# Elliotshui/ABRSimulator

Measured on AMD Instinct MI355X. Metric: env_steps_per_sec, higher is better.
Workload: dtype f64

## Files before the change

### abrsimulator_amd/csrc/abr_env.hip

```cpp
#include <hip/hip_runtime.h>

#include <climits>
#include <cmath>
#include <cstdarg>
#include <cstdio>
#include <cstdlib>
#include <cstring>
#include <new>
#include <type_traits>
#include <vector>

#include "abr_env.h"

#ifdef ABR_SPLIT_STAMPS
#include "abr_diag_stamps.h"
#else
#define ABR_STAMP(n)
#define ABR_STAMP_INIT()
#define ABR_STAMP_FLUSH()
#define ABR_WG_TIME(slot)
#define ABR_WG_WHERE(role)
#define K3_STAMP_DECL
#define K3_STAMP(n)
#define K3_STAMP_FLUSH()
#endif
#define ABR_RULE_KERNARG_OFFSET 592
#include "abr_lane_jump.h"
#include "abr_tick_tables.h"

static thread_local char g_err[512] = "";

static int fail(int code, const char *fmt, ...) {
    va_list ap;
    va_start(ap, fmt);
    vsnprintf(g_err, sizeof(g_err), fmt, ap);
    va_end(ap);
    return code;
}
#define HIP_TRY(expr)                                                                     \
    do {                                                                                  \
        hipError_t e__ = (expr);                                                          \
        if (e__ != hipSuccess)                                                            \
            return fail(ABR_E_HIP, "%s failed: %s", #expr, hipGetErrorString(e__));       \
    } while (0)

extern "C" int abr_abi_version(void) { return ABR_ABI_VERSION; }
extern "C" const char *abr_last_error(void) { return g_err; }

constexpr double kDt = 0.01;
constexpr int kFlagStartUp = 1, kFlagBufEmpty = 2, kFlagBufFull = 4;
constexpr int kFlagArmed = 8;

struct EnvParams {
    int32_t n_rates, video_length, max_ticks, auto_reset;
    int32_t play_ticks_per_chunk;
    int32_t n_intervals;
    int32_t t_block;
    int32_t n_traces;
    double chunk_length, max_buffer, start_up_length;
    double wr, wv, ws, wl;
    double sd;
    double ladder[ABR_MAX_RATES];
    int64_t n_lanes, lane_id_base;
    const double *G;
    const double *GP;
    const int32_t *interval_tick;
    const int32_t *avail_tick;
    abrx::DrainTab drain;
    const double *traces;
    const int64_t *trace_off;
    const int32_t *trace_len;
    double *buf, *last_bw, *hist_n, *hist_s;
    double *sd_lane, *pt_lane;
    const double *lane_speeds;
    int32_t speed_rows;
    int32_t *pl_left, *play_id;
    double *pt_sum;
    const double *br_table;
    long long *sumk;
    int32_t *k, *chunk_id, *n_su, *n_rb, *n_play, *j, *tpos, *trace_id, *offset0;
    int32_t *last_action, *n_su_obs, *n_rb_obs, *episode_no;
    uint8_t *flags, *done;
    uint8_t *action_hist;
    double *bw_hist;
    double *ep_qoe_terms;
    double *var_run;
    uint32_t *selfcheck_out;
    uint64_t sentinel;
    abrx::SpeedRuleBlock speed_rule;
};
static_assert(offsetof(EnvParams, speed_rule) == ABR_RULE_KERNARG_OFFSET, "abr_lane_jump.h reads the rule at this offset");
static_assert(sizeof(EnvParams) == 880, "the parameter block: 592 bytes + 288 of the speed rule");
static_assert(sizeof(abrx::SpeedRule) == sizeof(abr_speed_rule) &&
              offsetof(abrx::SpeedRule, lat_thr) == offsetof(abr_speed_rule, lat_thr) &&
              offsetof(abrx::SpeedRule, buf_thr) == offsetof(abr_speed_rule, buf_thr) &&
              offsetof(abrx::SpeedRule, speed) == offsetof(abr_speed_rule, speed), "abr_speed_rule: one layout");

constexpr uint32_t kTagMagic = 0x57524241u;
constexpr uint32_t kLayoutRev = 1;
struct WorkspaceTag {
    uint32_t magic, abi_version, layout_rev, n_rates;
    int64_t n_lanes;
    int32_t video_length, max_ticks, n_intervals, reserved_;
    uint64_t total_bytes;
    double chunk_length, interval, speed;
    uint8_t pad_[256 - 72];
};
static_assert(sizeof(WorkspaceTag) == 256, "the tag is one 256-byte block");
static_assert(sizeof(abrx::EpisodeSampler) == sizeof(abr_episode_sampler) &&
              offsetof(abrx::EpisodeSampler, pool) == offsetof(abr_episode_sampler, pool) &&
              offsetof(abrx::EpisodeSampler, n_pool) == offsetof(abr_episode_sampler, n_pool) &&
              offsetof(abrx::EpisodeSampler, offset_span) == offsetof(abr_episode_sampler, offset_span),
              "abr_episode_sampler: one layout");
static_assert(sizeof(abrx::EpisodeLedger) == sizeof(abr_episode_ledger) &&
              offsetof(abrx::EpisodeLedger, base) == offsetof(abr_episode_ledger, base_dev) &&
              offsetof(abrx::EpisodeLedger, rows) == offsetof(abr_episode_ledger, rows),
              "abr_episode_ledger: one layout");

struct abr_env {
    EnvParams p;
    abr_env_config cfg;
    size_t workspace_bytes;
    void *tag_dev;
    WorkspaceTag tag;
    int impl;
    int32_t *mpc_action;
    void *mpc_scratch;
    const double *pending_speeds;
    int32_t pending_speed_rows;
    bool pending_rule_on;
    abrx::SpeedRuleBlock pending_rule;
    bool speeds_dirty;
    const double *pending_br_table;
    bool br_table_dirty;
    bool armed;
    bool sampler_on;
    abrx::EpisodeSampler sampler;
    abrx::EpisodeLedger ledger;
};

static void apply_pending(abr_env *env) {
    if (env->br_table_dirty) { env->p.br_table = env->pending_br_table; env->br_table_dirty = false; }
    if (env->speeds_dirty) {
        env->p.lane_speeds = env->pending_speeds; env->p.speed_rows = env->pending_speed_rows;
        env->p.speed_rule = env->pending_rule;
        if (env->pending_rule_on) { env->p.lane_speeds = env->p.sd_lane; env->p.speed_rows = abrx::kSpeedRowsRule; }
        env->speeds_dirty = false;
    }
}

__device__ inline double chunk_bitrate(const EnvParams &p, int32_t chunk, int32_t rate) {
    return p.br_table ? p.br_table[(int64_t)chunk * p.n_rates + rate] : p.ladder[rate];
// ... 307 lines not shown
            bf = bufB >= max_buffer;
            be = bufB <= 0.0;
            buf = be ? 0.0 : bufB;
            su = su && !(buf >= sul);
            k += running ? 1 : 0;
            const bool next = running && (chunk_id < V) && (k < max_ticks);
            n_su += (next && su) ? 1 : 0;
            n_rb += (next && !su && be) ? 1 : 0;
            const bool call = done_dl && (k >= avail_k) && !bf;
            running = next && !call;
            const bool cross = (k == k_end);
            c = cross ? c_next : c;
            crossed = crossed || cross;
        }
        if (active) {
            s.buf = buf; s.dl = dl; s.c = c; s.k = k; s.chunk_id = chunk_id; s.n_su = n_su;
            s.n_rb = n_rb; s.n_play = n_play; s.n_dl = n_dl; s.avail_k = avail_k;
            s.su = su; s.be = be; s.bf = bf; s.done_dl = done_dl; s.running = running;
            s.sumk += (long long)sk;
            (void)crossed;
        }
    }

    if (touched) {
        lane_store(s, p, i);
        p.n_su_obs[i] = n_su_obs; p.n_rb_obs[i] = n_rb_obs; p.episode_no[i] = episode_no;
        p.last_bw[i] = last_bw; p.hist_n[i] = hist_n; p.hist_s[i] = hist_s; p.var_run[i] = var_run;
        p.done[i] = done;
        if (MODE != 0) {
            for (int32_t t = step_idx; t < n_total; t++) {
                const int64_t o = (int64_t)t * p.n_lanes + i;
                if (reward_out) reward_out[o] = 0.0f;
                if (done_out) done_out[o] = done;
                if ((MODE == 2 || MODE == 4) && actions_out) actions_out[o] = -1;
                if (obs_out)
                    write_obs(s, p, i, obs_out + (int64_t)t * ABR_OBS_DIM * p.n_lanes, last_bw);
            }
        }
    }
}

using abrx::LaneJ;

__device__ inline abrx::Tables make_tables(const EnvParams &p, bool cascade = true) {
    abrx::Tables t;
    t.G = p.G; t.interval_tick = p.interval_tick; t.avail_tick = p.avail_tick;
    t.L = p.chunk_length; t.sd = p.sd; t.max_buffer = p.max_buffer;
    t.start_up_length = p.start_up_length; t.V = p.video_length; t.max_ticks = p.max_ticks;
    t.per_lane_speed = p.lane_speeds != nullptr;
    t.speed_rows = p.lane_speeds ? p.speed_rows : 0;
    t.speed_stride = p.n_lanes; t.speeds = p.lane_speeds;
    t.drain = p.drain;
    if (p.lane_speeds || !cascade) t.drain.n = 0;
#ifdef ABR_NO_DRAIN_CASCADE
    t.drain.n = 0;
#endif
    return t;
}

__device__ inline void lanej_load(LaneJ &s, const EnvParams &p, int64_t i) {
    s.buf = p.buf[i]; s.sumk = p.sumk[i];
    s.k = p.k[i]; s.chunk_id = p.chunk_id[i]; s.n_su = p.n_su[i]; s.n_rb = p.n_rb[i];
    s.n_play = p.n_play[i]; s.cur.j = p.j[i]; s.cur.tpos = p.tpos[i];
    s.last_action = p.last_action[i];
    const uint8_t f = p.flags[i];
    s.su = f & kFlagStartUp; s.be = f & kFlagBufEmpty; s.bf = f & kFlagBufFull;
    const int32_t c = s.chunk_id < p.video_length ? s.chunk_id : p.video_length;
    s.avail_k = p.avail_tick[c];
    if (p.lane_speeds) { s.sd = p.sd_lane[i]; s.pt = p.pt_lane[i]; } else { s.sd = p.sd; s.pt = 0.0; }
    s.lane = i; s.pl_left = 0; s.play_id = 0; s.pt_sum = 0.0;
    if (p.lane_speeds && p.speed_rows >= 2) { s.pl_left = p.pl_left[i]; s.play_id = p.play_id[i]; s.pt_sum = p.pt_sum[i]; }
}

__device__ inline void lanej_store(const LaneJ &s, const EnvParams &p, int64_t i) {
    p.buf[i] = s.buf; p.sumk[i] = s.sumk;
    p.k[i] = s.k; p.chunk_id[i] = s.chunk_id; p.n_su[i] = s.n_su; p.n_rb[i] = s.n_rb;
    p.n_play[i] = s.n_play; p.j[i] = s.cur.j; p.tpos[i] = s.cur.tpos; p.last_action[i] = s.last_action;
    p.flags[i] = (uint8_t)((s.su ? kFlagStartUp : 0) | (s.be ? kFlagBufEmpty : 0) |
                           (s.bf ? kFlagBufFull : 0) | kFlagArmed);
    if (p.lane_speeds) { p.sd_lane[i] = s.sd; p.pt_lane[i] = s.pt; }
    if (p.lane_speeds && p.speed_rows >= 2) { p.pl_left[i] = s.pl_left; p.play_id[i] = s.play_id; p.pt_sum[i] = s.pt_sum; }
}

#ifndef ABR_NO_NT_STORES
#define ABR_OUT(ref, val) __builtin_nontemporal_store((val), &(ref))
#else
#define ABR_OUT(ref, val) ((ref) = (val))
#endif

__device__ inline void write_obs_j(const LaneJ &s, const EnvParams &p, int64_t i, float *obs,
                                   double last_bw) {
    if (!obs) return;
    const int64_t n = p.n_lanes;
    ABR_OUT(obs[ABR_OBS_CHUNK_ID * n + i], (float)s.chunk_id);
    ABR_OUT(obs[ABR_OBS_LAST_BITRATE * n + i], (float)s.last_action);
    ABR_OUT(obs[ABR_OBS_LAST_BANDWIDTH * n + i], (float)last_bw);
    ABR_OUT(obs[ABR_OBS_BUFFER_LEVEL * n + i], (float)s.buf);
    ABR_OUT(obs[ABR_OBS_GLOBAL_TIME * n + i], (float)p.G[s.k]);
    ABR_OUT(obs[ABR_OBS_PLAY_TIME * n + i], (float)(p.lane_speeds ? s.pt : p.GP[s.n_play]));
    ABR_OUT(obs[ABR_OBS_REBUFFER_TIME * n + i], (float)p.G[s.n_rb]);
    ABR_OUT(obs[ABR_OBS_STARTUP_TIME * n + i], (float)p.G[s.n_su]);
}

__device__ inline void write_obs_vals(const LaneJ &s, const EnvParams &p, int64_t i, float *obs, double last_bw,
                                      double g_k, double g_play, double g_rb, double g_su) {
    if (!obs) return;
// ... 187 lines not shown
}

__global__ void observe_f64_kernel(EnvParams p, double *__restrict__ out) {
    const int64_t i = (int64_t)blockIdx.x * blockDim.x + threadIdx.x;
    if (i >= p.n_lanes) return;
    const int64_t n = p.n_lanes;
    out[ABR_F64_GLOBAL_TIME * n + i] = p.G[p.k[i]];
    out[ABR_F64_REBUFFER_TIME * n + i] = p.G[p.n_rb[i]];
    out[ABR_F64_STARTUP_TIME * n + i] = p.G[p.n_su[i]];
    int32_t P = p.play_ticks_per_chunk;
    const bool sched = p.lane_speeds && p.speed_rows >= 2;
    if (p.lane_speeds) {
        double x = 0.0; int32_t a = 0;
        abrx::chain<abrx::STOP_GE>(x, p.sd_lane[i], p.chunk_length, p.max_ticks + 1, a);
        P = a > 0 ? a : 1;
        out[ABR_F64_PLAY_TIME * n + i] = p.pt_lane[i];
        out[ABR_F64_AVERAGE_LATENCY * n + i] =
            sched ? avg_latency_sched(p.pt_lane[i], p.sumk[i], p.pt_sum[i], p.n_play[i])
                  : avg_latency_from(p.sd_lane[i], p.pt_lane[i], p.sumk[i], p.n_play[i]);
    } else {
        out[ABR_F64_PLAY_TIME * n + i] = p.GP[p.n_play[i]];
        out[ABR_F64_AVERAGE_LATENCY * n + i] = lane_avg_latency(p, p.sumk[i], p.n_play[i]);
    }
    out[ABR_F64_BUFFER_LEVEL * n + i] = p.buf[i];
    if (sched) {
        const int32_t pl = p.pl_left[i];
        double x = 0.0; int32_t a = 0;
        abrx::chain<abrx::STOP_GE>(x, p.sd_lane[i], 1.0e300, pl > 0 ? P - pl : 0, a);
        out[ABR_F64_PLAY_LENGTH * n + i] = x;
    } else if (p.lane_speeds) {
        double x = 0.0; int32_t a = 0;
        abrx::chain<abrx::STOP_GE>(x, p.sd_lane[i], 1.0e300, p.n_play[i] % P, a);
        out[ABR_F64_PLAY_LENGTH * n + i] = x;
    } else {
        out[ABR_F64_PLAY_LENGTH * n + i] = p.GP[p.n_play[i] % P];
    }
    out[ABR_F64_LAST_BANDWIDTH * n + i] = p.last_bw[i];
    out[ABR_F64_CHUNK_ID * n + i] = (double)p.chunk_id[i];
    out[ABR_F64_PLAY_ID * n + i] = sched ? (double)p.play_id[i] : (double)(p.n_play[i] / P);
    out[ABR_F64_LAST_BITRATE * n + i] = (double)p.last_action[i];
    out[ABR_F64_FLAGS * n + i] = (double)p.flags[i];
    out[ABR_F64_HIST_N * n + i] = p.hist_n[i];
    out[ABR_F64_HIST_SUM_INV * n + i] = p.hist_s[i];
    out[ABR_F64_TICK * n + i] = (double)p.k[i];
    out[ABR_F64_DOWNLOAD_TIME * n + i] = 0.0;
}

static size_t align_up(size_t x, size_t a) { return (x + a - 1) / a * a; }
static size_t mpc_scratch_bytes_max(size_t n_lanes) {
    return n_lanes * ((size_t)ABR_MAX_HORIZON * sizeof(double) + 2 * sizeof(int32_t));
}

struct Layout {
    size_t G, GP, interval_tick, avail_tick;
    size_t f64_state, i64_state, i32_state, u8_state, action_hist, bw_hist, ep_terms;
    size_t mpc_action, mpc_scratch;
    size_t tag;
    size_t total;
    int32_t max_ticks, n_intervals;
};

static double min_episode_ticks(const abr_env_config *c) {
    return ((double)c->video_length + 1.0) * ceil(c->chunk_length / kDt);
}
static double default_max_ticks(const abr_env_config *c) {
    double per_chunk = ceil(c->chunk_length / kDt);
    double mt = 32.0 * c->video_length * per_chunk;
    if (mt > 16.0e6) mt = 16.0e6;
    if (mt < 2.0 * min_episode_ticks(c)) mt = 2.0 * min_episode_ticks(c);
    if (mt < 1024) mt = 1024;
    return mt;
}

static int validate_cfg(const abr_env_config *c) {
    if (!c) return fail(ABR_E_INVALID, "config is NULL");
    if (c->n_rates < 1 || c->n_rates > ABR_MAX_RATES)
        return fail(ABR_E_INVALID, "n_rates %d outside 1..%d", c->n_rates, ABR_MAX_RATES);
    if (c->video_length < 1 || c->video_length > 65535)
        return fail(ABR_E_INVALID, "video_length %d outside 1..65535", c->video_length);
    if (!(c->chunk_length > 0) || !(c->interval > 0) || !(c->speed > 0))
        return fail(ABR_E_INVALID, "chunk_length, interval and speed must be > 0");
    if (!(c->max_buffer > 0)) return fail(ABR_E_INVALID, "max_buffer must be > 0");
    if (!(c->start_up_length >= 0)) return fail(ABR_E_INVALID, "start_up_length must be >= 0");
    if (c->chunk_length / kDt > 1.0e6)
        return fail(ABR_E_UNSUPPORTED, "chunk_length %g s is more than 1e6 ticks", c->chunk_length);
    for (int r = 0; r < c->n_rates; r++)
        if (!(c->ladder[r] > 0)) return fail(ABR_E_INVALID, "ladder[%d] must be > 0", r);
    return ABR_OK;
}

static int compute_layout(const abr_env_config *c, int64_t n_lanes, Layout *L) {
    int rc = validate_cfg(c);
    if (rc) return rc;
    if (n_lanes < 1) return fail(ABR_E_INVALID, "n_lanes must be >= 1");
    const double mtd = c->max_ticks > 0 ? (double)c->max_ticks : default_max_ticks(c);
    if (mtd > 256.0e6)
        return fail(ABR_E_UNSUPPORTED, "video_length %d x chunk_length %g s needs a %g-entry tick table",
                    c->video_length, c->chunk_length, mtd);
    if (mtd < min_episode_ticks(c))
        return fail(ABR_E_INVALID, "max_ticks %g is below (video_length + 1) * ceil(chunk_length / dt) = %g: "
                    "every lane would end in ABR_DONE_TIMEOUT", mtd, min_episode_ticks(c));
    const int32_t mt = (int32_t)mtd;
    double n_iv = (double)mt * kDt / c->interval + 4.0;
    if (n_iv > 32.0e6)
        return fail(ABR_E_UNSUPPORTED, "interval %g s needs a %g-entry tick table", c->interval, n_iv);
    L->max_ticks = mt;
    L->n_intervals = (int32_t)n_iv;
    size_t o = 0;
    const size_t A = 256;
    size_t N = (size_t)n_lanes, V = (size_t)c->video_length;
    L->G = o; o = align_up(o + sizeof(double) * ((size_t)mt + 2), A);
    L->GP = o; o = align_up(o + sizeof(double) * ((size_t)mt + 2), A);
    L->interval_tick = o; o = align_up(o + sizeof(int32_t) * ((size_t)L->n_intervals + 8), A);
    L->avail_tick = o; o = align_up(o + sizeof(int32_t) * (V + 2), A);
    L->f64_state = o; o = align_up(o + sizeof(double) * 8 * N, A);
    L->i64_state = o; o = align_up(o + sizeof(long long) * 1 * N, A);
    L->i32_state = o; o = align_up(o + sizeof(int32_t) * 15 * N, A);
    L->u8_state = o; o = align_up(o + 2 * N, A);
    L->action_hist = o; o = align_up(o + V * N, A);
    L->bw_hist = o; o = align_up(o + sizeof(double) * V * N, A);
    L->ep_terms = o; o = align_up(o + sizeof(double) * 4 * N, A);
    L->mpc_action = o; o = align_up(o + sizeof(int32_t) * N, A);
    L->mpc_scratch = o; o = align_up(o + mpc_scratch_bytes_max(N), A);
    L->tag = o; o = align_up(o + sizeof(WorkspaceTag), A);
    L->total = o;
    return ABR_OK;
}

extern "C" int abr_env_workspace_bytes(const abr_env_config *cfg, int64_t n_lanes,
                                       size_t *bytes_out) {
    Layout L;
    int rc = compute_layout(cfg, n_lanes, &L);
    if (rc) return rc;
    if (!bytes_out) return fail(ABR_E_INVALID, "bytes_out is NULL");
    *bytes_out = L.total;
    return ABR_OK;
}

extern "C" int abr_env_create(const abr_env_config *cfg, const double *traces_dev,
                              const int64_t *trace_off_dev, const int32_t *trace_len_dev,
                              int32_t n_traces, int64_t n_lanes, void *workspace_dev,
                              size_t workspace_bytes, void *stream, abr_env **env_out) {
    Layout L;
    int rc = compute_layout(cfg, n_lanes, &L);
    if (rc) return rc;
    if (!env_out) return fail(ABR_E_INVALID, "env_out is NULL");
    if (!traces_dev || !trace_off_dev || !trace_len_dev || n_traces < 1)
        return fail(ABR_E_INVALID, "trace arrays missing");
    if (!workspace_dev || ((uintptr_t)workspace_dev & 255))
        return fail(ABR_E_WORKSPACE, "workspace must be non-NULL and 256-B aligned");
    if (workspace_bytes < L.total)
        return fail(ABR_E_WORKSPACE, "workspace has %zu bytes, need %zu", workspace_bytes, L.total);

    const int32_t mt = L.max_ticks;
    abrx::TickTables tt = abrx::build_tick_tables(cfg->interval, cfg->chunk_length, cfg->speed,
                                                  cfg->video_length, mt, L.n_intervals);
    std::vector<double> &G = tt.G, &GP = tt.GP;
    std::vector<int32_t> &itick = tt.interval_tick, &atick = tt.avail_tick;
    const double sd = tt.sd;
    const int32_t P = tt.play_ticks_per_chunk;
    int32_t t_block = tt.min_interval_ticks < 128 ? tt.min_interval_ticks : 128;
    if (t_block < 1) t_block = 1;
    if (P == INT_MAX)
        return fail(ABR_E_UNSUPPORTED, "max_ticks %d too small to play one chunk", mt);

    abr_env *e = new (std::nothrow) abr_env;
    if (!e) return fail(ABR_E_INVALID, "out of host memory");
    memset(e, 0, sizeof(*e));
    e->cfg = *cfg;
    e->impl = 3;
    e->workspace_bytes = L.total;
    EnvParams &p = e->p;
    p.n_rates = cfg->n_rates; p.video_length = cfg->video_length; p.max_ticks = mt;
    p.auto_reset = cfg->auto_reset; p.play_ticks_per_chunk = P; p.n_intervals = L.n_intervals;
    p.t_block = t_block; p.n_traces = n_traces;
    p.chunk_length = cfg->chunk_length; p.max_buffer = cfg->max_buffer;
    p.start_up_length = cfg->start_up_length;
    p.wr = cfg->rebuffer_weight; p.wv = cfg->variance_weight; p.ws = cfg->startup_weight;
    p.wl = cfg->latency_weight; p.sd = sd;
    for (int r = 0; r < ABR_MAX_RATES; r++) p.ladder[r] = cfg->ladder[r];
    p.n_lanes = n_lanes; p.lane_id_base = 0;
    char *w = (char *)workspace_dev;
    p.G = (const double *)(w + L.G); p.GP = (const double *)(w + L.GP);
    p.interval_tick = (const int32_t *)(w + L.interval_tick);
    p.avail_tick = (const int32_t *)(w + L.avail_tick);
    p.drain = abrx::make_drain_tab(sd, cfg->max_buffer + cfg->chunk_length);
    p.traces = traces_dev; p.trace_off = trace_off_dev; p.trace_len = trace_len_dev;
    const size_t N = (size_t)n_lanes;
    double *f = (double *)(w + L.f64_state);
    p.buf = f; p.last_bw = f + N; p.hist_n = f + 2 * N; p.hist_s = f + 3 * N;
    p.sd_lane = f + 4 * N; p.pt_lane = f + 5 * N; p.pt_sum = f + 6 * N; p.var_run = f + 7 * N; p.lane_speeds = nullptr;
    p.speed_rows = 1;
    p.speed_rule = abrx::SpeedRuleBlock{};
    p.sumk = (long long *)(w + L.i64_state);
    int32_t *q = (int32_t *)(w + L.i32_state);
    p.k = q; p.chunk_id = q + N; p.n_su = q + 2 * N; p.n_rb = q + 3 * N; p.n_play = q + 4 * N;
    p.j = q + 5 * N; p.tpos = q + 6 * N; p.trace_id = q + 7 * N; p.offset0 = q + 8 * N;
    p.last_action = q + 9 * N; p.n_su_obs = q + 10 * N; p.n_rb_obs = q + 11 * N;
    p.episode_no = q + 12 * N; p.pl_left = q + 13 * N; p.play_id = q + 14 * N;
    uint8_t *u = (uint8_t *)(w + L.u8_state);
    p.flags = u; p.done = u + N;
    p.action_hist = (uint8_t *)(w + L.action_hist);
    p.bw_hist = (double *)(w + L.bw_hist);
    p.ep_qoe_terms = (double *)(w + L.ep_terms);
    e->mpc_action = (int32_t *)(w + L.mpc_action);
    e->mpc_scratch = (void *)(w + L.mpc_scratch);

    hipStream_t st = (hipStream_t)stream;
    hipError_t he;
#define UP(dst, vec)                                                                           \
    he = hipMemcpyAsync((void *)(dst), (vec).data(), (vec).size() * sizeof((vec)[0]),          \
                        hipMemcpyHostToDevice, st);                                            \
    if (he != hipSuccess) { delete e; return fail(ABR_E_HIP, "table upload: %s", hipGetErrorString(he)); }
    UP(p.G, G) UP(p.GP, GP) UP(p.interval_tick, itick) UP(p.avail_tick, atick)
#undef UP
    he = hipMemsetAsync(w + L.f64_state, 0, L.total - L.f64_state, st);
    if (he == hipSuccess) he = hipMemsetAsync(p.done, ABR_DONE_EPISODE, N, st);
    {
        WorkspaceTag &tg = e->tag;
        memset(&tg, 0, sizeof(tg));
        tg.magic = kTagMagic; tg.abi_version = ABR_ABI_VERSION; tg.layout_rev = kLayoutRev; tg.n_rates = (uint32_t)cfg->n_rates;
        tg.n_lanes = n_lanes; tg.video_length = cfg->video_length; tg.max_ticks = mt; tg.n_intervals = L.n_intervals;
        tg.total_bytes = L.total; tg.chunk_length = cfg->chunk_length; tg.interval = cfg->interval; tg.speed = cfg->speed;
        e->tag_dev = w + L.tag;
        if (he == hipSuccess) he = hipMemcpyAsync(e->tag_dev, &tg, sizeof(tg), hipMemcpyHostToDevice, st);
    }
    if (he == hipSuccess) he = hipStreamSynchronize(st);
    if (he != hipSuccess) { delete e; return fail(ABR_E_HIP, "workspace init: %s", hipGetErrorString(he)); }
    *env_out = e;
    return ABR_OK;
}

extern "C" int abr_env_destroy(abr_env *env) {
    delete env;
    return ABR_OK;
}

extern "C" int abr_env_has_impl(int32_t impl) {
    switch (impl) {
    case 0: case 1: case 2: case 3: case 5: return 1;
#ifdef ABR_WITH_ASYNC
    case 4: return 1;
#endif
#ifdef ABR_WITH_RING
    case 6: case 7: return 1;
#endif
    default: return 0;
    }
}

enum Feature { kLaneSpeeds, kSpeedRule, kRuleRollout, kMpcRollout, kPolicyRollout };
static const struct { unsigned impls; const char *what; } kFeatures[] = {
    {0xFDu, "per-lane speeds and speed schedules need the event-driven kernels"},
    {0x2Du, "a speed rule needs the event-driven kernels that read it"},
    {0x0Bu, "rule rollouts run on the one-thread-per-lane kernels"},
    {0xFDu, "the fused MPC rollout needs the event-driven kernels"},
    {0xFDu, "the fused policy rollout needs the event-driven kernels"},
};

static int require(Feature f, int impl) {
    const unsigned ok = kFeatures[f].impls;
    if (ok >> impl & 1u) return ABR_OK;
    int ks[8], n = 0, len = 0;
    for (int k = 0; k < 8; k++)
        if ((ok >> k & 1u) && abr_env_has_impl(k)) ks[n++] = k;
    char list[48] = "";
    for (int i = 0; i < n; i++)
// ... 1795 lines not shown
```

### abrsimulator_amd/csrc/abr_env_roles.h

```cpp
#ifndef ABR_ENV_ROLES_H
#define ABR_ENV_ROLES_H


#ifndef ABR_SPLIT3_CASCADE
#define ABR_SPLIT3_CASCADE 0
#endif
#ifndef ABR_PRIO_D
#define ABR_PRIO_D 2
#endif
#ifndef ABR_PRIO_P
#define ABR_PRIO_P 1
#endif
#ifndef ABR_PRIO_S
#define ABR_PRIO_S 0
#endif

struct SplitMail {
    double dl[2][64];
    int32_t n_dl[2][64], k_start[2][64], step[2][64], action[2][64], avail_next[2][64], flags[2][64];
    int32_t fb_step[2][64], fb_k[2][64], fb_chunk[2][64], fb_episode[2][64], fb_alive[2][64];
    double fb_buf[2][64];
    int32_t fb_pf[2][64];
    int32_t any_alive[2];
};
// ... 246 lines not shown
    int at = 0;
    p_unwords(k, at, v, p);
}

__device__ __forceinline__ double player_latency(const EnvParams &p, const LaneJ &s) {
    return !p.lane_speeds ? lane_avg_latency(p, s.sumk, s.n_play)
           : (p.speed_rows >= 2 ? avg_latency_sched(s.pt, s.sumk, s.pt_sum, s.n_play)
                                : avg_latency_from(s.sd, s.pt, s.sumk, s.n_play));
}

__device__ __forceinline__ void player_feedback(SplitMail &m, const PVars &v, int32_t n_total, int cb) {
    const int l = threadIdx.x & 63;
    const bool more = v.b_alive && v.b_step < n_total;
    m.fb_step[cb][l] = v.b_step; m.fb_k[cb][l] = v.s.k; m.fb_chunk[cb][l] = v.s.chunk_id;
    m.fb_episode[cb][l] = v.episode_no; m.fb_alive[cb][l] = more ? 1 : 0;
    m.fb_buf[cb][l] = v.s.buf; m.fb_pf[cb][l] = (v.s.su ? 1 : 0) | (v.s.be ? 2 : 0);
    const bool any = __any(more) != 0;
    if (l == 0) m.any_alive[cb] = any ? 1 : 0;
}

__device__ __forceinline__ void player_clear(PVars &v, const EnvParams &p) {
    LaneJ &s = v.s;
    s.buf = 0.0; s.sd = 0.0; s.pt = 0.0; s.pt_sum = 0.0; s.sumk = 0;
    s.k = 0; s.chunk_id = 0; s.n_su = 0; s.n_rb = 0; s.n_play = 0; s.avail_k = 0; s.last_action = -1;
    s.pl_left = 0; s.play_id = 0; s.su = false; s.be = false; s.bf = false;
    s.cur.j = 0; s.cur.tpos = 0; s.cur.tlen = 1; s.cur.trace = p.traces;
    s.lane = (int64_t)blockIdx.x * 64 + (threadIdx.x & 63);
    v.episode_no = 0; v.b_step = 0; v.b_alive = false; v.was_done = true;
}

__device__ __forceinline__ void role_p3_begin(PVars &v, const EnvParams &p) {
    const int64_t i = (int64_t)blockIdx.x * 64 + (threadIdx.x & 63);
    player_clear(v, p);
    if (i < p.n_lanes) {
        v.was_done = p.done[i] != 0;
        lanej_load(v.s, p, i);
        v.episode_no = p.episode_no[i];
        v.b_alive = !v.was_done;
    }
    ABR_STAMP_INIT();
}

template <int MODE, class M2>
__device__ __forceinline__ void role_p3_pre(PVars &v, const EnvParams &p, SplitMail &m, M2 &m2,
                                            int32_t n_total, int32_t t, int cb2) {
    const int l = threadIdx.x & 63;
    const int cb = t & 1, pb = (t + 1) & 1;
    const abrx::Tables tb = make_tables(p, ABR_SPLIT3_CASCADE != 0);
    const bool speeds = p.lane_speeds != nullptr;
    LaneJ &s = v.s;
    int32_t meta = 0;
    ABR_STAMP(8);
    if (v.b_alive && v.b_step < n_total && t >= 1) {
        int32_t fl = m.flags[pb][l];
        int32_t r_step = m.step[pb][l], r_k = m.k_start[pb][l], r_a = m.action[pb][l], r_ndl = m.n_dl[pb][l],
                r_avail = m.avail_next[pb][l];
        double r_dl = m.dl[pb][l];
        asm volatile("" : "+v"(fl), "+v"(r_step), "+v"(r_k), "+v"(r_a), "+v"(r_ndl), "+v"(r_avail), "+v"(r_dl));
        if ((fl & kRecValid) && r_step == v.b_step && r_k == s.k) {
            const int32_t a = r_a;
            meta = kS3Valid | (a & 0xff);
            m2.step[cb2][l] = v.b_step;
            if (fl & kRecBadAct) {
                meta |= kS3Bad;
                v.b_alive = false;
            } else {
                abrx::Download d;
                d.dl = r_dl; d.n_dl = r_ndl; d.hit = (fl & kRecHit) != 0;
                const abrx::StepResult sr = abrx::lanej_after_download(s, tb, d, r_avail, a);
                if (sr.hit) meta |= kS3Hit;
                if (sr.ended) meta |= kS3Ended;
                if (sr.timeout) meta |= kS3Timeout;
                m2.dl[cb2][l] = d.dl; m2.n_dl[cb2][l] = d.n_dl;
                m2.nrb_r[cb2][l] = s.n_rb; m2.nsu_r[cb2][l] = s.n_su;
                if (sr.ended || sr.timeout) {
                    m2.lat[cb2][l] = player_latency(p, s);
                    if (p.auto_reset && sr.ended) {
                        abrx::lanej_init_player(s, tb);
                        v.episode_no++;
                        meta |= kS3Reset;
                        if (!abrx::lanej_wait_call(s, tb)) { meta |= kS3Timeout2; v.b_alive = false; }
                    } else v.b_alive = false;
                }
                m2.buf[cb2][l] = s.buf; m2.k[cb2][l] = s.k; m2.nplay_o[cb2][l] = s.n_play;
                m2.nrb_o[cb2][l] = s.n_rb; m2.nsu_o[cb2][l] = s.n_su;
                if (speeds) m2.pt[cb2][l] = s.pt;
            }
            v.b_step++;
        }
    }
    ABR_STAMP(13);
    m2.meta[cb2][l] = meta;
    player_feedback(m, v, n_total, cb);
    ABR_STAMP(17);
}

__device__ __forceinline__ void role_p3_end(const PVars &v, const EnvParams &p) {
    const int64_t i = (int64_t)blockIdx.x * 64 + (threadIdx.x & 63);
    ABR_STAMP_FLUSH();
    if (i < p.n_lanes && !v.was_done) lanej_store_player(v.s, p, i);
}

struct SVars {
    double last_bw, hist_n, hist_s, g_su_obs, g_rb_obs;
    double var_run;
    double o_buf, o_pt;
    int32_t o_chunk, o_last, o_k, o_nplay, o_nrb, o_nsu;
    int32_t n_su_obs, n_rb_obs, episode_no, s_next;
    int32_t a_next, a_chunk, a_ep;
    int32_t last_cb;
    uint8_t done;
    bool was_done;
};
__device__ __forceinline__ void s_park(uint32_t (*area)[64], const SVars &v) {
    ParkWords k; k.n = 0;
    pw_f64(k, v.last_bw); pw_f64(k, v.hist_n); pw_f64(k, v.hist_s); pw_f64(k, v.g_su_obs); pw_f64(k, v.g_rb_obs);
    pw_f64(k, v.o_buf); pw_f64(k, v.o_pt);
    pw_i32(k, v.o_chunk); pw_i32(k, v.o_last); pw_i32(k, v.o_k); pw_i32(k, v.o_nplay); pw_i32(k, v.o_nrb);
    pw_i32(k, v.o_nsu); pw_i32(k, v.n_su_obs); pw_i32(k, v.n_rb_obs); pw_i32(k, v.episode_no); pw_i32(k, v.s_next);
    pw_i32(k, v.a_next); pw_i32(k, v.a_chunk); pw_i32(k, v.a_ep); pw_i32(k, v.last_cb);
    pw_i32(k, (int32_t)v.done | (v.was_done ? 0x100 : 0));
    pw_f64(k, v.var_run); pw_i32(k, 0);
// ... 450 lines not shown
```

### abrsimulator_amd/csrc/abr_lane_jump.h

```cpp
#ifndef ABR_LANE_JUMP_H
#define ABR_LANE_JUMP_H

#include <math.h>

#include "abr_exact_jump.h"

#ifndef ABR_STAMP
#define ABR_STAMP(n)
#endif

namespace abrx {

constexpr double kTickDt = 0.01;
#ifndef ABR_K_DRAIN_TAIL
#define ABR_K_DRAIN_TAIL 16
#endif
constexpr int kPrologue = 16;
#ifndef ABR_PCHUNKS
#define ABR_PCHUNKS 12
#endif
#ifndef ABR_PCHECK
#define ABR_PCHECK 0x892
#endif
constexpr int kPChunks = ABR_PCHUNKS;
constexpr int kPCheck = ABR_PCHECK;

struct SpeedRule {
    int32_t n_lat, n_buf;
    double lat_thr[4], buf_thr[4];
    double speed[5][5];
};

ABR_HD double speed_rule_eval(const SpeedRule &r, double lat, double buf) {
    int32_t i = 0, j = 0;
    for (int32_t q = 0; q < r.n_lat; q++) i += lat >= r.lat_thr[q] ? 1 : 0;
    for (int32_t q = 0; q < r.n_buf; q++) j += buf >= r.buf_thr[q] ? 1 : 0;
    return r.speed[i][j];
}

constexpr int32_t kSpeedRowsRule = 0x7fffffff;

struct SpeedRuleBlock {
    SpeedRule rule;
    double *log;
    int32_t log_rows, reserved_;
};

struct Tables {
    const double *G;
    const int32_t *interval_tick;
    const int32_t *avail_tick;
    double L, sd, max_buffer, start_up_length;
    int32_t V, max_ticks;
    bool per_lane_speed;
    int32_t speed_rows;
    int64_t speed_stride;
    const double *speeds;
    const SpeedRuleBlock *rule = nullptr;
    DrainTab drain;
};

struct Cursor {
    int32_t j;
    int32_t tpos;
    int32_t tlen;
    const double *trace;
};

struct LaneJ {
    double buf;
    double sd;
    double pt;
    long long sumk;
    int32_t k, chunk_id, n_su, n_rb, n_play, avail_k, last_action;
    bool su, be, bf;
    Cursor cur;
    int32_t pl_left, play_id;
    double pt_sum;
    int64_t lane;
};

ABR_HD void cursor_init(Cursor &c, int32_t offset0) {
    c.j = 0;
    c.tpos = offset0 % c.tlen;
}

ABR_HD void lanej_init_player(LaneJ &s, const Tables &t) {
    s.buf = 0.0; s.sumk = 0;
    s.k = 0; s.chunk_id = 0; s.n_su = 1; s.n_rb = 0; s.n_play = 0;
    s.last_action = -1;
    s.su = true; s.be = true; s.bf = false;
    s.avail_k = t.avail_tick[0];
    s.pt = 0.0;
    s.pl_left = 0; s.play_id = 0; s.pt_sum = 0.0;
}

ABR_HD void lanej_init(LaneJ &s, const Tables &t, int32_t offset0) {
    lanej_init_player(s, t);
    cursor_init(s.cur, offset0);
}

ABR_HD void lanej_play(LaneJ &s, const Tables &t, int32_t a) {
    if (!t.per_lane_speed || a <= 0) return;
    int32_t done = 0;
    double x = s.pt;
    chain<STOP_GE>(x, s.sd, 1.0e300, a, done);
    s.pt = x;
}

constexpr int kDrainTail = ABR_K_DRAIN_TAIL;
ABR_HD bool drain_to_zero(double &b_io, double sd, int32_t m, int32_t &a_out) {
    ChainState cs;
    cs.x = b_io; cs.eb = -1;
    const double tail = (double)kDrainTail * sd;
    int32_t a = 0;
    bool below = false;
    while (a < m && !below) a += chain_segment<STOP_LE>(cs, -sd, tail, m - a, below);
    double b = cs.x;
    ABR_STAMP(24);
#ifdef ABR_DRAIN_HOOK
    const int32_t a_seg = a;
#endif
#if defined(__HIP_DEVICE_COMPILE__)
#pragma unroll 1
#endif
    while (a < m && b > 0.0) { b = b - sd; a++; }
    ABR_STAMP(25);
#ifdef ABR_DRAIN_HOOK
    ABR_DRAIN_HOOK(a > 0 && b <= 0.0, a - a_seg);
#endif
    b_io = b; a_out = a;
    return a > 0 && b <= 0.0;
}

ABR_HD bool lanej_drain(const Tables &t, double &b_io, double sd, int32_t m, int32_t &a_out) {
    if (t.drain.n > 0 && !wave_any(!(b_io < t.drain.top))) {
        const bool zero = drain_cascade(t.drain, sd, b_io, m, a_out);
        ABR_STAMP(24);
        return zero;
    }
    return drain_to_zero(b_io, sd, m, a_out);
}

ABR_HD void sched_begin_chunk(LaneJ &s, const Tables &t, int32_t k, double b) {
    double v;
    if (t.speed_rows == kSpeedRowsRule) {
#if defined(__HIP_DEVICE_COMPILE__) && defined(ABR_RULE_KERNARG_OFFSET)
        auto kp = __builtin_amdgcn_kernarg_segment_ptr();
        asm volatile("" : "+s"(kp));
        const SpeedRuleBlock &rb = *(const SpeedRuleBlock *)((const char *)kp + ABR_RULE_KERNARG_OFFSET);
#else
        const SpeedRuleBlock &rb = *t.rule;
#endif
        v = speed_rule_eval(rb.rule, t.G[k] - s.pt, b);
        if (s.play_id < rb.log_rows) rb.log[(int64_t)s.play_id * t.speed_stride + s.lane] = v;
    } else {
        const int32_t row = s.play_id < t.speed_rows ? s.play_id : t.speed_rows - 1;
        v = t.speeds[(int64_t)row * t.speed_stride + s.lane];
    }
    s.sd = v * kTickDt;
    double x = 0.0;
    int32_t a = 0;
    chain<STOP_GE>(x, s.sd, t.L, t.max_ticks + 1, a);
    s.pl_left = a > 0 ? a : 1;
}

ABR_HD void sched_played(LaneJ &s, const Tables &t, int32_t a) {
    if (a <= 0) return;
    s.pt_sum += (double)a * s.pt + s.sd * (double)(((long long)a * (a - 1)) / 2);
    int32_t done = 0;
    double x = s.pt;
    chain<STOP_GE>(x, s.sd, 1.0e300, a, done);
    s.pt = x;
    s.pl_left -= a;
    if (s.pl_left == 0) s.play_id++;
}

template <int STOP>
ABR_HD bool sched_drain(LaneJ &s, const Tables &t, double &b, double thr, int32_t m, int32_t &a_out) {
    int32_t a_tot = 0;
    bool hit = false;
    while (a_tot < m && !hit) {
        if (s.pl_left == 0) sched_begin_chunk(s, t, s.k + a_tot, b);
        const int32_t run = (m - a_tot < s.pl_left) ? m - a_tot : s.pl_left;
        int32_t a = 0;
        if (STOP == STOP_LE) hit = drain_to_zero(b, s.sd, run, a);
        else hit = chain<STOP_LT>(b, -s.sd, thr, run, a);
        sched_played(s, t, a);
        a_tot += a;
    }
    a_out = a_tot;
    return hit;
}

ABR_HD void lanej_idle(LaneJ &s, const Tables &t, int32_t m) {
    if (m <= 0) return;
    if (s.su && s.buf >= t.start_up_length) s.su = false;
    ABR_STAMP(23);
    if (s.su) {
        s.n_su += m;
    } else if (s.be) {
        s.n_rb += m;
    } else {
        int32_t a = 0;
        double b = s.buf;
        bool zero;
        if (t.speed_rows >= 2) zero = sched_drain<STOP_LE>(s, t, b, 0.0, m, a);
        else { zero = lanej_drain(t, b, s.sd, m, a); lanej_play(s, t, a); }
        s.n_play += a;
        s.sumk += (long long)a * s.k + ((long long)a * (a - 1)) / 2;
        if (zero) { b = 0.0; s.be = true; s.n_rb += (m - a + 1); }
        s.buf = b;
        s.bf = b >= t.max_buffer;
    }
    s.k += m;
}

ABR_HD bool lanej_wait_call(LaneJ &s, const Tables &t) {
    const int32_t mt = t.max_ticks;
    if (s.k >= s.avail_k && !s.bf) return true;
    int32_t w = s.avail_k - s.k;
    if (w < 0) w = 0;
    if (w > mt - s.k) w = mt - s.k;
    lanej_idle(s, t, w);
    if (s.k >= mt) return false;
    if (s.bf) {
        if (s.su || s.be) {
            if (s.su) s.n_su += mt - s.k; else s.n_rb += mt - s.k;
            s.k = mt;
            return false;
        }
        int32_t a = 0;
        double b = s.buf;
        bool cleared;
        if (t.speed_rows >= 2) cleared = sched_drain<STOP_LT>(s, t, b, t.max_buffer, mt - s.k, a);
        else { cleared = chain<STOP_LT>(b, -s.sd, t.max_buffer, mt - s.k, a); lanej_play(s, t, a); }
        s.n_play += a;
        s.sumk += (long long)a * s.k + ((long long)a * (a - 1)) / 2;
        s.k += a;
        s.be = b <= 0.0;
        if (s.be) { b = 0.0; s.n_rb += 1; }
        s.buf = b;
        s.bf = !cleared;
        if (!cleared) return false;
    }
    return true;
}

struct StepResult {
    double bw;
    bool hit;
    bool ended;
    bool timeout;
};

constexpr int kCatch = 4;
struct StepStart {
    double c;
    double bw_next;
    int32_t ke;
    int32_t ke_next;
// ... 90 lines not shown
        const int32_t left = ke - kk;
        const int32_t n1 = left > 0 ? left : 0;
        const int32_t a = n1 & 7, q1 = n1 >> 3;
        const double c2 = bw_next * kTickDt;
        const int32_t room2 = (ke_next < mt ? ke_next : mt) - ke;
        double x = 0.0, xb = 0.0;
        int32_t T = 0;
#if defined(__HIP_DEVICE_COMPILE__)
#pragma unroll
#endif
        for (int i = 0; i < 7; i++) x = (i < a) ? x + c : x;
#if defined(__HIP_DEVICE_COMPILE__)
#pragma unroll
#endif
        for (int q = 0; q < kPChunks; q++) {
            const double cq = (q < q1) ? c : c2;
#if defined(__HIP_DEVICE_COMPILE__)
#pragma unroll
#endif
            for (int i = 0; i < 8; i++) x = x + cq;
            if ((kPCheck >> q) & 1) {
                const int32_t Tq = a + 8 * (q + 1);
                const bool ok = (x < target) & ((Tq <= n1) | (Tq - n1 < room2));
                xb = ok ? x : xb;
                T = ok ? Tq : T;
            }
        }
        cs.x = xb;
        const bool crossed = T > n1;
        kk += T;
        c = crossed ? c2 : c;
        ke = crossed ? (ke_next < mt ? ke_next : mt) : ke;
        s.j += crossed ? 1 : 0;
        s.tpos = crossed ? tn : s.tpos;
    }
    while (!hit && kk < mt) {
        const bool adv = kk >= ke;
        c = adv ? bw_next * kTickDt : c;
        ke = adv ? (ke_next < mt ? ke_next : mt) : ke;
        s.j += adv ? 1 : 0;
        s.tpos = adv ? tn : s.tpos;
        cs.eb = adv ? -1 : cs.eb;
        tn = (s.tpos + 1 == s.tlen) ? 0 : s.tpos + 1;
        bw_next = s.trace[(uint32_t)tn];
        ke_next = t.interval_tick[(uint32_t)(s.j + 2)];
        kk += chain_segment<STOP_GE>(cs, c, target, ke - kk, hit);
    }
    Download d;
    d.dl = cs.x; d.n_dl = kk - k; d.hit = hit;
    return d;
}

ABR_HD StepResult lanej_after_download(LaneJ &s, const Tables &t, const Download &d,
                                       int32_t avail_next, int32_t action) {
    StepResult r;
    r.bw = 0.0; r.hit = false; r.ended = false; r.timeout = false;
    const int32_t mt = t.max_ticks;
    const bool hit = d.hit;
    const int32_t n_dl = d.n_dl;
    const double g_ndl = t.G[n_dl];
    lanej_idle(s, t, hit ? n_dl - 1 : n_dl);
    ABR_STAMP(10);
    if (!hit) { r.timeout = true; return r; }
    const bool playing = !(s.be || s.su);
    double b = s.buf + t.L;
    if (playing) {
        s.sumk += s.k; s.n_play++;
        if (t.speed_rows >= 2) {
            if (s.pl_left == 0) sched_begin_chunk(s, t, s.k, b);
            b = b - s.sd;
            sched_played(s, t, 1);
        } else { b = b - s.sd; lanej_play(s, t, 1); }
    }
    s.bf = b >= t.max_buffer;
    s.be = b <= 0.0;
    if (s.be) b = 0.0;
    s.buf = b;
    s.su = s.su && !(b >= t.start_up_length);
    s.k++;
    r.hit = true;
    r.bw = d.dl / g_ndl;
    s.last_action = action;
    s.chunk_id++;
    s.avail_k = avail_next;
    r.ended = s.chunk_id >= t.V;
    r.timeout = !r.ended && s.k >= mt;
    ABR_STAMP(11);
    if (!r.ended && !r.timeout) {
        s.n_su += s.su ? 1 : 0;
        s.n_rb += (!s.su && s.be) ? 1 : 0;
        r.timeout = !lanej_wait_call(s, t);
    }
    ABR_STAMP(12);
    return r;
}

ABR_HD bool lanej_gate_possible(double buf, bool su, bool be, int32_t n_dl, const Tables &t) {
    return !su && !be && !t.per_lane_speed && (buf + t.L) - (double)n_dl * t.sd >= t.max_buffer - 1.0e-6;
}
ABR_HD bool lanej_predict_next_call(double buf, int32_t k, int32_t n_dl, int32_t avail_next, const Tables &t,
                                    int32_t &k_next, double *buf_next = nullptr) {
    const int32_t mt = t.max_ticks;
    double b = buf;
    int32_t a = 0;
    if (n_dl > 1 && lanej_drain(t, b, t.sd, n_dl - 1, a)) return false;
    b = b + t.L;
    b = b - t.sd;
    if (b <= 0.0) return false;
    bool bf = b >= t.max_buffer;
    k += n_dl;
    if (k >= mt) return false;
    if (!(k >= avail_next && !bf)) {
        int32_t w = avail_next - k;
        if (w < 0) w = 0;
// ... 446 lines not shown
```

### abrsimulator_amd/csrc/abr_tick_tables.h

```cpp
#ifndef ABR_TICK_TABLES_H
#define ABR_TICK_TABLES_H

#include <climits>
#include <cstdint>
#include <vector>

namespace abrx {

struct TickTables {
    std::vector<double> G, GP;
    std::vector<int32_t> interval_tick;
    std::vector<int32_t> avail_tick;
    int32_t play_ticks_per_chunk;
    int32_t min_interval_ticks;
    double sd;
};

inline TickTables build_tick_tables(double interval, double chunk_length, double speed,
                                    int32_t video_length, int32_t max_ticks, int32_t n_intervals) {
    const double dt = 0.01;
    TickTables t;
    const int32_t mt = max_ticks;
    t.sd = speed * dt;
    t.G.resize((size_t)mt + 2);
    t.GP.resize((size_t)mt + 2);
    double g = 0.0, gp = 0.0;
    for (int32_t n = 0; n < mt + 2; n++) {
        t.G[n] = g; t.GP[n] = gp;
        g += dt;
        gp += t.sd;
    }
    t.interval_tick.assign((size_t)n_intervals + 8, INT_MAX);
    {
        int64_t jcur = 0;
        for (int32_t k = 0; k <= mt && jcur < n_intervals + 8; k++) {
            int64_t idx = (int64_t)(t.G[k] / interval);
            while (jcur <= idx && jcur < n_intervals + 8) t.interval_tick[jcur++] = k;
        }
    }
    t.min_interval_ticks = INT_MAX;
    for (size_t j = 0; j + 1 < t.interval_tick.size() && t.interval_tick[j + 1] != INT_MAX; j++) {
        int32_t len = t.interval_tick[j + 1] - t.interval_tick[j];
        if (len < t.min_interval_ticks) t.min_interval_ticks = len;
    }
    if (t.min_interval_ticks == INT_MAX) t.min_interval_ticks = mt;
    t.avail_tick.assign((size_t)video_length + 2, INT_MAX);
    {
        int64_t ccur = 0;
        for (int32_t k = 0; k <= mt && ccur < video_length; k++) {
            int64_t avail = (int64_t)(t.G[k] / chunk_length) - 1;
            while (ccur <= avail && ccur < video_length) t.avail_tick[ccur++] = k;
        }
    }
    t.play_ticks_per_chunk = INT_MAX;
    for (int32_t n = 1; n < mt + 2; n++)
        if (t.GP[n] >= chunk_length) { t.play_ticks_per_chunk = n; break; }
    return t;
}

}
#endif
```

Measured before the change: 12.39 billion.

## Add precomputed dry-out threshold table to resolve buffer drain in closed form

Builds a host-side table of exact floating-point buffer thresholds, one per tick count it takes repeated subtraction of the drain step to reach zero, and uploads it with the other tick tables. Idle drains then look up the tick count with a reciprocal multiply and three compares instead of walking the drain loop or cascade, falling back when a lane is outside the table or the rebuffer does not happen inside the window. The table probe is also issued early in the role kernel, before the record loads, so its memory latency can overlap with them. This costs an extra 8192-entry table, a larger kernel argument block, and a new correctness dependency on the exact-rounding table construction.

```diff
diff --git a/abrsimulator_amd/csrc/abr_env.hip b/abrsimulator_amd/csrc/abr_env.hip
--- a/abrsimulator_amd/csrc/abr_env.hip
+++ b/abrsimulator_amd/csrc/abr_env.hip
@@ -24,7 +24,7 @@
 #define K3_STAMP(n)
 #define K3_STAMP_FLUSH()
 #endif
-#define ABR_RULE_KERNARG_OFFSET 592
+#define ABR_RULE_KERNARG_OFFSET 616
 #include "abr_lane_jump.h"
 #include "abr_tick_tables.h"
 
@@ -67,6 +67,9 @@
     const int32_t *interval_tick;
     const int32_t *avail_tick;
     abrx::DrainTab drain;
+    const double *dry;
+    int32_t dry_n, dry_reserved_;
+    double dry_rcp;
     const double *traces;
     const int64_t *trace_off;
     const int32_t *trace_len;
@@ -90,14 +93,14 @@
     abrx::SpeedRuleBlock speed_rule;
 };
 static_assert(offsetof(EnvParams, speed_rule) == ABR_RULE_KERNARG_OFFSET, "abr_lane_jump.h reads the rule at this offset");
-static_assert(sizeof(EnvParams) == 880, "the parameter block: 592 bytes + 288 of the speed rule");
+static_assert(sizeof(EnvParams) == 904, "the parameter block: 616 bytes + 288 of the speed rule");
 static_assert(sizeof(abrx::SpeedRule) == sizeof(abr_speed_rule) &&
               offsetof(abrx::SpeedRule, lat_thr) == offsetof(abr_speed_rule, lat_thr) &&
               offsetof(abrx::SpeedRule, buf_thr) == offsetof(abr_speed_rule, buf_thr) &&
               offsetof(abrx::SpeedRule, speed) == offsetof(abr_speed_rule, speed), "abr_speed_rule: one layout");
 
 constexpr uint32_t kTagMagic = 0x57524241u;
-constexpr uint32_t kLayoutRev = 1;
+constexpr uint32_t kLayoutRev = 2;
 struct WorkspaceTag {
     uint32_t magic, abi_version, layout_rev, n_rates;
     int64_t n_lanes;
@@ -511,6 +514,11 @@
     t.speed_stride = p.n_lanes; t.speeds = p.lane_speeds;
     t.drain = p.drain;
     if (p.lane_speeds || !cascade) t.drain.n = 0;
+    t.dry = p.dry; t.dry_rcp = p.dry_rcp;
+    t.dry_n = p.lane_speeds ? 0 : p.dry_n;
+#ifdef ABR_NO_DRY_TABLE
+    t.dry_n = 0;
+#endif
 #ifdef ABR_NO_DRAIN_CASCADE
     t.drain.n = 0;
 #endif
@@ -804,7 +812,7 @@
 }
 
 struct Layout {
-    size_t G, GP, interval_tick, avail_tick;
+    size_t G, GP, interval_tick, avail_tick, dry;
     size_t f64_state, i64_state, i32_state, u8_state, action_hist, bw_hist, ep_terms;
     size_t mpc_action, mpc_scratch;
     size_t tag;
@@ -865,6 +873,7 @@
     L->GP = o; o = align_up(o + sizeof(double) * ((size_t)mt + 2), A);
     L->interval_tick = o; o = align_up(o + sizeof(int32_t) * ((size_t)L->n_intervals + 8), A);
     L->avail_tick = o; o = align_up(o + sizeof(int32_t) * (V + 2), A);
+    L->dry = o; o = align_up(o + sizeof(double) * (size_t)abrx::kDryCapacity, A);
     L->f64_state = o; o = align_up(o + sizeof(double) * 8 * N, A);
     L->i64_state = o; o = align_up(o + sizeof(long long) * 1 * N, A);
     L->i32_state = o; o = align_up(o + sizeof(int32_t) * 15 * N, A);
@@ -937,6 +946,13 @@
     p.interval_tick = (const int32_t *)(w + L.interval_tick);
     p.avail_tick = (const int32_t *)(w + L.avail_tick);
     p.drain = abrx::make_drain_tab(sd, cfg->max_buffer + cfg->chunk_length);
+    abrx::DryTable dry = abrx::build_dry_table(sd, cfg->max_buffer + cfg->chunk_length);
+    {
+        const char *sw = getenv("ABR_DRY_TABLE");
+        if (sw && sw[0] == '0' && sw[1] == 0) dry.n = 0;
+    }
+    std::vector<double> &dryv = dry.theta;
+    p.dry = (const double *)(w + L.dry); p.dry_n = dry.n; p.dry_reserved_ = 0; p.dry_rcp = dry.rcp;
     p.traces = traces_dev; p.trace_off = trace_off_dev; p.trace_len = trace_len_dev;
     const size_t N = (size_t)n_lanes;
     double *f = (double *)(w + L.f64_state);
@@ -964,7 +980,7 @@
     he = hipMemcpyAsync((void *)(dst), (vec).data(), (vec).size() * sizeof((vec)[0]),          \
                         hipMemcpyHostToDevice, st);                                            \
     if (he != hipSuccess) { delete e; return fail(ABR_E_HIP, "table upload: %s", hipGetErrorString(he)); }
-    UP(p.G, G) UP(p.GP, GP) UP(p.interval_tick, itick) UP(p.avail_tick, atick)
+    UP(p.G, G) UP(p.GP, GP) UP(p.interval_tick, itick) UP(p.avail_tick, atick) UP(p.dry, dryv)
 #undef UP
     he = hipMemsetAsync(w + L.f64_state, 0, L.total - L.f64_state, st);
     if (he == hipSuccess) he = hipMemsetAsync(p.done, ABR_DONE_EPISODE, N, st);
diff --git a/abrsimulator_amd/csrc/abr_env_roles.h b/abrsimulator_amd/csrc/abr_env_roles.h
--- a/abrsimulator_amd/csrc/abr_env_roles.h
+++ b/abrsimulator_amd/csrc/abr_env_roles.h
@@ -322,6 +322,7 @@
     int32_t meta = 0;
     ABR_STAMP(8);
     if (v.b_alive && v.b_step < n_total && t >= 1) {
+        abrx::DryProbe pre = abrx::dry_probe(tb, s.buf);
         int32_t fl = m.flags[pb][l];
         int32_t r_step = m.step[pb][l], r_k = m.k_start[pb][l], r_a = m.action[pb][l], r_ndl = m.n_dl[pb][l],
                 r_avail = m.avail_next[pb][l];
@@ -337,7 +338,8 @@
             } else {
                 abrx::Download d;
                 d.dl = r_dl; d.n_dl = r_ndl; d.hit = (fl & kRecHit) != 0;
-                const abrx::StepResult sr = abrx::lanej_after_download(s, tb, d, r_avail, a);
+                asm volatile("" : "+v"(pre.th0), "+v"(pre.th1), "+v"(pre.th2));
+                const abrx::StepResult sr = abrx::lanej_after_download(s, tb, d, r_avail, a, &pre);
                 if (sr.hit) meta |= kS3Hit;
                 if (sr.ended) meta |= kS3Ended;
                 if (sr.timeout) meta |= kS3Timeout;
diff --git a/abrsimulator_amd/csrc/abr_lane_jump.h b/abrsimulator_amd/csrc/abr_lane_jump.h
--- a/abrsimulator_amd/csrc/abr_lane_jump.h
+++ b/abrsimulator_amd/csrc/abr_lane_jump.h
@@ -58,6 +58,9 @@
     const double *speeds;
     const SpeedRuleBlock *rule = nullptr;
     DrainTab drain;
+    const double *dry = nullptr;
+    int32_t dry_n = 0;
+    double dry_rcp = 0.0;
 };
 
 struct Cursor {
@@ -133,13 +136,47 @@
     return a > 0 && b <= 0.0;
 }
 
-ABR_HD bool lanej_drain(const Tables &t, double &b_io, double sd, int32_t m, int32_t &a_out) {
+struct DryProbe {
+    double th0, th1, th2;
+    int32_t k0;
+};
+ABR_HD DryProbe dry_probe(const Tables &t, double x) {
+    DryProbe p;
+    p.k0 = (int32_t)clamp0(sat_i32(x * t.dry_rcp), t.dry_n);
+    const double *q = t.dry + (uint32_t)p.k0;
+    p.th0 = q[0]; p.th1 = q[1]; p.th2 = q[2];
+    return p;
+}
+ABR_HD bool dry_covered(const Tables &t, const DryProbe &p) { return p.k0 <= t.dry_n - 3; }
+ABR_HD int32_t dry_ticks(const DryProbe &p, double x) {
+    return p.k0 + (x > p.th0 ? 1 : 0) + (x > p.th1 ? 1 : 0) + (x > p.th2 ? 1 : 0);
+}
+
+ABR_HD bool lanej_drain_plain(const Tables &t, double &b_io, double sd, int32_t m, int32_t &a_out) {
     if (t.drain.n > 0 && !wave_any(!(b_io < t.drain.top))) {
         const bool zero = drain_cascade(t.drain, sd, b_io, m, a_out);
         ABR_STAMP(24);
         return zero;
     }
     return drain_to_zero(b_io, sd, m, a_out);
+}
+
+ABR_HD bool lanej_drain(const Tables &t, double &b_io, double sd, int32_t m, int32_t &a_out,
+                        const DryProbe *pre = nullptr) {
+    if (t.dry_n > 0) {
+        const DryProbe pr = pre ? *pre : dry_probe(t, b_io);
+        if (!wave_any(!dry_covered(t, pr))) {
+            const int32_t T = dry_ticks(pr, b_io);
+            const bool dry = (T >= 1) & (T <= m);
+            double b = b_io;
+            int32_t a = 0;
+            lanej_drain_plain(t, b, sd, dry ? 0 : m, a);
+            b_io = dry ? 0.0 : b;
+            a_out = dry ? T : a;
+            return dry;
+        }
+    }
+    return lanej_drain_plain(t, b_io, sd, m, a_out);
 }
 
 ABR_HD void sched_begin_chunk(LaneJ &s, const Tables &t, int32_t k, double b) {
@@ -193,7 +230,7 @@
     return hit;
 }
 
-ABR_HD void lanej_idle(LaneJ &s, const Tables &t, int32_t m) {
+ABR_HD void lanej_idle(LaneJ &s, const Tables &t, int32_t m, const DryProbe *pre = nullptr) {
     if (m <= 0) return;
     if (s.su && s.buf >= t.start_up_length) s.su = false;
     ABR_STAMP(23);
@@ -206,7 +243,7 @@
         double b = s.buf;
         bool zero;
         if (t.speed_rows >= 2) zero = sched_drain<STOP_LE>(s, t, b, 0.0, m, a);
-        else { zero = lanej_drain(t, b, s.sd, m, a); lanej_play(s, t, a); }
+        else { zero = lanej_drain(t, b, s.sd, m, a, pre); lanej_play(s, t, a); }
         s.n_play += a;
         s.sumk += (long long)a * s.k + ((long long)a * (a - 1)) / 2;
         if (zero) { b = 0.0; s.be = true; s.n_rb += (m - a + 1); }
@@ -403,14 +440,14 @@
 }
 
 ABR_HD StepResult lanej_after_download(LaneJ &s, const Tables &t, const Download &d,
-                                       int32_t avail_next, int32_t action) {
+                                       int32_t avail_next, int32_t action, const DryProbe *pre = nullptr) {
     StepResult r;
     r.bw = 0.0; r.hit = false; r.ended = false; r.timeout = false;
     const int32_t mt = t.max_ticks;
     const bool hit = d.hit;
     const int32_t n_dl = d.n_dl;
     const double g_ndl = t.G[n_dl];
-    lanej_idle(s, t, hit ? n_dl - 1 : n_dl);
+    lanej_idle(s, t, hit ? n_dl - 1 : n_dl, pre);
     ABR_STAMP(10);
     if (!hit) { r.timeout = true; return r; }
     const bool playing = !(s.be || s.su);
diff --git a/abrsimulator_amd/csrc/abr_tick_tables.h b/abrsimulator_amd/csrc/abr_tick_tables.h
--- a/abrsimulator_amd/csrc/abr_tick_tables.h
+++ b/abrsimulator_amd/csrc/abr_tick_tables.h
@@ -2,7 +2,9 @@
 #define ABR_TICK_TABLES_H
 
 #include <climits>
+#include <cmath>
 #include <cstdint>
+#include <limits>
 #include <vector>
 
 namespace abrx {
@@ -58,5 +60,40 @@
     return t;
 }
 
+constexpr int32_t kDryCapacity = 8192;
+constexpr int32_t kDrySlack = 8;
+constexpr int32_t kDryPad = 3;
+
+struct DryTable {
+    std::vector<double> theta;
+    int32_t n = 0;
+    double rcp = 0.0;
+};
+
+inline DryTable build_dry_table(double sd, double max_level, int32_t capacity = kDryCapacity, double window = 0.25) {
+    DryTable t;
+    t.theta.assign((size_t)(capacity > 0 ? capacity : 0), std::numeric_limits<double>::infinity());
+    if (!(sd > 0.0) || !(max_level > 0.0) || !(sd < 1.0e300) || !(max_level < 1.0e300) || !(sd >= 1.0e-300)) return t;
+    const double need = std::ceil(max_level / sd) + (double)kDrySlack;
+    if (!(need + (double)kDryPad + 1.0 <= (double)capacity)) return t;
+    const int32_t n = (int32_t)need;
+    t.theta[0] = 0.0;
+    for (int32_t k = 1; k <= n; k++) {
+        const double prev = t.theta[k - 1];
+        double x = prev + sd;
+        int guard = 0;
+        while (x - sd > prev && guard++ < 64) x = std::nextafter(x, -std::numeric_limits<double>::infinity());
+        while (std::nextafter(x, std::numeric_limits<double>::infinity()) - sd <= prev && guard++ < 64)
+            x = std::nextafter(x, std::numeric_limits<double>::infinity());
+        const bool settled = (x - sd <= prev) && (std::nextafter(x, std::numeric_limits<double>::infinity()) - sd > prev);
+        const double dev = x - (double)k * sd;
+        if (!settled || !(x > prev) || !((dev < 0.0 ? -dev : dev) < window * sd)) return t;
+        t.theta[k] = x;
+    }
+    t.n = n;
+    t.rcp = 1.0 / sd;
+    return t;
+}
+
 }
 #endif
```

Result: slower. 11.88 billion (-4.2%).
